# instadeepai/FrameDiPT

Hardware: AMD Instinct MI355X
Metric: residue*diffusion-steps/sec (higher is better)
Workload: dtype fp16

## Files before the change

framedipt_amd/csrc/ipa_proj2.hip:

```cpp
#include <type_traits>

#include "common.hpp"
#include "kernels.hpp"

#define P2_K 256
#define P2_KS (P2_K / 16)
#define P2_WBLK (4 * P2_KS * 1024)
#define P2_XROW (P2_K * 2)
#define P2_LDS (2 * P2_WBLK)

typedef const __attribute__((address_space(3))) float* p2_lds_f32;

#define P2S_HALF 32768
#define P2S_STAGE (2 * P2S_HALF)
#define P2S_BIAS_OFF (2 * P2S_STAGE)
__host__ __device__ __forceinline__ int p2p_src_col(int n) {
  const int c = n >> 7, col = n & 127;
  if (c < 4) {
    if (col < 72) { const int vh = col / 36, r = col % 36; return 192 + (r % 3) * 160 + (2 * c + vh) * 20 + 8 + r / 3; }
    if (col < 120) { const int r = col - 72, kh = r / 24, q = r % 24; return 192 + (q % 3) * 160 + (2 * c + kh) * 20 + q / 3; }
    return -1;
  }
  if (c > 5 || col >= 96) return -1;
  const int hq = col / 24, r = col % 24;
  return (r % 3) * 64 + (4 * (c - 4) + hq) * 8 + r / 3;
}
#define P2P_COLS 768
typedef __attribute__((address_space(3))) f32x4* p2_lds_f32x4w;
typedef __attribute__((address_space(3))) u16x8* p2_lds_u16x8w;
typedef const __attribute__((address_space(3))) unsigned* p2_lds_u32;

__device__ __forceinline__ void p2_kpf_units(const ProjArgs& a, const float (&kv)[24], bool lv, int b, int h, int key, int ntl) {
#pragma unroll
  for (int un = 0; un < 8; ++un) {
    const int f = un >> 1, hf = un & 1;
    unsigned short o[8];
    if (f == 3 && hf == 1) {
      float kn = 0.f;
      if (lv)
#pragma unroll
        for (int c = 0; c < 24; ++c) kn = fmaf(kv[c], kv[c], kn);
      const float m = lv ? a.res_mask[(long)b * a.N + key] : 0.f;
      const float t0 = fmaxf(-0.5f * a.gamma[h] * kn, -65000.f);
      const unsigned short p0 = f2f16(t0);
      const float t1 = t0 - f162f(p0);
      const unsigned short p1 = f2f16(t1);
      const unsigned short p2 = f2f16(t1 - f162f(p1));
      o[0] = f2f16(2.f * m); o[1] = f2f16(m); o[2] = f2f16(lv ? 0.f : -60000.f); o[3] = p0; o[4] = p1; o[5] = p2; o[6] = o[7] = 0;
    } else {
      const int c0 = f < 2 ? 8 * hf : 16;
      const bool lo = f == 1 || (f == 2 && hf == 1);
#pragma unroll
      for (int e = 0; e < 8; ++e) {
        const float x = lv ? kv[c0 + e] : 0.f;
        const unsigned short xh = f2f16(x);
        o[e] = lo ? f2f16(x - f162f(xh)) : xh;
      }
    }
    const u32x4 val = {o[0] | ((unsigned)o[1] << 16), o[2] | ((unsigned)o[3] << 16), o[4] | ((unsigned)o[5] << 16), o[6] | ((unsigned)o[7] << 16)};
    *(u32x4*)(a.kpf + ((((((long)b * a.H + h) * ntl + (key >> 5)) * FD_KPF_FRAGS + f) * 64 + hf * 32 + (key & 31)) << 3)) = val;
  }
}

template <class RQ>
__device__ __forceinline__ void p2_points_walk(const ProjArgs& a, const hx8 (&Af)[P2_KS], const hx8 (&Al)[P2_KS], int n_class, int nq, int walker,
                                               int n_walkers, unsigned lds0, unsigned fr, RQ& request_half) {
  const int tid = threadIdx.x, lane = tid & 63, wave = tid >> 6, li = lane & 31, hi = lane >> 5;
  const int M = a.B * a.N, m0 = blockIdx.x * 256, H = a.H, ntl = a.Np >> 5, ks = a.Np >> 4;
  auto tile_at = [&](int col, int rg) { return lds0 + (unsigned)(col * 1024 + ((rg ^ (col & 63)) << 4)); };
  auto rotate = [&](int row, float px, float py, float pz, float* g3) {
    float R[12];
#pragma unroll
    for (int i = 0; i < 12; ++i) R[i] = *(p2_lds_f32)(unsigned long)(fr + 4 * (i * 256 + row));
    g3[0] = R[0] * px + R[1] * py + R[2] * pz + R[9];
    g3[1] = R[3] * px + R[4] * py + R[5] * pz + R[10];
    g3[2] = R[6] * px + R[7] * py + R[8] * pz + R[11];
  };
  for (int k = walker; k < n_class; k += n_walkers) {
    const int c = nq + k;
    const bool frames = k == walker && tid < 256;
    f32x4 fq = {0.f, 0.f, 0.f, 0.f};
    float ft[3] = {0.f, 0.f, 0.f};
    if (frames) {
      const int gr = m0 + tid < M ? m0 + tid : M - 1;
      fq = *(const f32x4*)(a.quat + (long)gr * 4);
#pragma unroll
      for (int d = 0; d < 3; ++d) ft[d] = a.trans[(long)gr * 3 + d];
    }
    __syncthreads();
    request_half(c, 0, 0);
    request_half(c, 1, 1);
#pragma unroll 1
    for (int half = 0; half < 2; ++half) {
      if (half == 0) __builtin_amdgcn_s_waitcnt(0x0F78);
      else __builtin_amdgcn_s_waitcnt(0x0F70);
      if (half == 0 && frames) {
        const float w = fq[0], x = fq[1], y = fq[2], z = fq[3];
        float R[9];
        R[0] = w * w + x * x - y * y - z * z; R[1] = 2 * x * y - 2 * w * z; R[2] = 2 * x * z + 2 * w * y;
        R[3] = 2 * x * y + 2 * w * z; R[4] = w * w - x * x + y * y - z * z; R[5] = 2 * y * z - 2 * w * x;
        R[6] = 2 * x * z - 2 * w * y; R[7] = 2 * y * z + 2 * w * x; R[8] = w * w - x * x - y * y + z * z;
#pragma unroll
        for (int i = 0; i < 12; ++i) *(__attribute__((address_space(3))) float*)(unsigned long)(fr + 4 * (i * 256 + tid)) = i < 9 ? R[i] : ft[i - 9];
        if (walker == 0 && m0 + tid < M)
#pragma unroll
          for (int i = 0; i < 9; ++i) a.rot[(long)(m0 + tid) * 9 + i] = R[i];
      }
      __syncthreads();
      f32x16 acc[2];
#pragma unroll
      for (int j = 0; j < 2; ++j) {
#pragma unroll
        for (int r = 0; r < 16; ++r) acc[j][r] = 0.f;
        const unsigned wbh = lds0 + half * P2S_STAGE + j * (P2_KS * 1024) + lane * 16, wbl = wbh + P2S_HALF;
        constexpr int DEPTH = 3;
        hx8 wh[DEPTH], wl[DEPTH];
#pragma unroll
        for (int s = 0; s < DEPTH - 1; ++s) { wh[s] = fd_frag(wbh + s * 1024); wl[s] = fd_frag(wbl + s * 1024); }
        __builtin_amdgcn_sched_barrier(0);
#pragma unroll
        for (int s = 0; s < P2_KS; ++s) {
          if (s + DEPTH - 1 < P2_KS) {
            wh[(s + DEPTH - 1) % DEPTH] = fd_frag(wbh + (s + DEPTH - 1) * 1024);
            wl[(s + DEPTH - 1) % DEPTH] = fd_frag(wbl + (s + DEPTH - 1) * 1024);
          }
          const hx8 h = wh[s % DEPTH], l = wl[s % DEPTH];
          acc[j] = fd_mfma32(Af[s], l, acc[j]);
          acc[j] = fd_mfma32(Al[s], h, acc[j]);
          acc[j] = fd_mfma32(Af[s], h, acc[j]);
          __builtin_amdgcn_sched_barrier(0);
        }
      }
      float bv[2];
#pragma unroll
      for (int j = 0; j < 2; ++j) bv[j] = *(p2_lds_f32)(unsigned long)(lds0 + P2S_BIAS_OFF + 4 * (c * 128 + 64 * half + 32 * j + li));
      __syncthreads();
#pragma unroll
      for (int j = 0; j < 2; ++j)
#pragma unroll
        for (int g = 0; g < 4; ++g) {
          const f32x4 v = {acc[j][4 * g] + bv[j], acc[j][4 * g + 1] + bv[j], acc[j][4 * g + 2] + bv[j], acc[j][4 * g + 3] + bv[j]};
          *(p2_lds_f32x4w)(unsigned long)tile_at(64 * half + 32 * j + li, 8 * wave + 2 * g + hi) = v;
        }
    }
    __syncthreads();
    auto tv = [&](int row, int col) { return *(p2_lds_f32)(unsigned long)(tile_at(col, row >> 2) + 4 * (row & 3)); };
    int tid = threadIdx.x;
    asm volatile("" : "+v"(tid));
    if (k < 4) {
      {
        const int row = tid & 255, kh = tid >> 8, m = m0 + row;
        if (m < M) {
          const int b = m / a.N, key = m - b * a.N;
          float kv[24];
#pragma unroll
          for (int e = 0; e < 8; ++e) {
            const int col = 72 + 24 * kh + 3 * e;
            rotate(row, tv(row, col), tv(row, col + 1), tv(row, col + 2), kv + 3 * e);
          }
          p2_kpf_units(a, kv, true, b, 2 * k + kh, key, ntl);
        }
        const int npad = a.Np - a.N;
        if (npad > 0)
          for (int bs = m0 / a.N; bs < a.B && bs * a.N < m0 + 256; ++bs) {
            const int end = bs * a.N + a.N - 1;
            if (end < m0 || end >= m0 + 256) continue;
            float z[24];
#pragma unroll
            for (int q = 0; q < 24; ++q) z[q] = 0.f;
#pragma unroll 1
            for (int u = tid; u < 2 * npad; u += 512) p2_kpf_units(a, z, false, bs, 2 * k + (u & 1), a.N + (u >> 1), ntl);
          }
      }
#pragma unroll 1
      for (int t = tid; t < 64 * 24; t += 512) {
        const int k4 = t & 63, rest = t >> 6, vh = rest / 12, e = rest - 12 * vh, mg = m0 + 4 * k4;
        if (mg >= M) continue;
        const int b = mg / a.N, key = mg - b * a.N, pp = (key & ~15) + fd_perm16(key & 15), h = 2 * k + vh;
        f32x4 pc[3];
#pragma unroll
        for (int d = 0; d < 3; ++d) pc[d] = *(fd_lds_f32x4)(unsigned long)tile_at(36 * vh + 3 * e + d, k4);
        unsigned short vhs[3][4], vls[3][4];
#pragma unroll
        for (int q = 0; q < 4; ++q) {
          float g3[3];
          rotate(4 * k4 + q, pc[0][q], pc[1][q], pc[2][q], g3);
#pragma unroll
          for (int d = 0; d < 3; ++d) {
            const unsigned short vh16 = f2h(g3[d]);
            vhs[d][q] = vh16;
            vls[d][q] = f2h(g3[d] - h2f(vh16));
          }
        }
#pragma unroll
        for (int d = 0; d < 3; ++d) {
          const int rw = 3 * e + d, rl = 36 + rw;
          const long bh3 = ((long)b * H + h) * 3;
          const long oh = ((((bh3 + (rw >> 5)) * ks + (pp >> 4)) * 64 + ((pp >> 3) & 1) * 32 + (rw & 31)) << 3) + (pp & 7);
          const long ol = ((((bh3 + (rl >> 5)) * ks + (pp >> 4)) * 64 + ((pp >> 3) & 1) * 32 + (rl & 31)) << 3) + (pp & 7);
          *(u32x2*)(a.vpt + oh) = u32x2{vhs[d][0] | ((unsigned)vhs[d][1] << 16), vhs[d][2] | ((unsigned)vhs[d][3] << 16)};
          *(u32x2*)(a.vpt + ol) = u32x2{vls[d][0] | ((unsigned)vls[d][1] << 16), vls[d][2] | ((unsigned)vls[d][3] << 16)};
        }
      }
    } else {
#pragma unroll 1
      for (int t = tid; t < 1024; t += 512) {
        const int row = t & 255, hq = t >> 8, m = m0 + row;
        if (m >= M) continue;
        float g[24];
#pragma unroll
        for (int e = 0; e < 8; ++e) {
          const int col = 24 * hq + 3 * e;
          rotate(row, tv(row, col), tv(row, col + 1), tv(row, col + 2), g + 3 * e);
        }
        float* dst = a.qp + ((long)m * H * 8 + (4 * (k - 4) + hq) * 8) * 3;
#pragma unroll
        for (int v = 0; v < 6; ++v) *(f32x4*)(dst + 4 * v) = f32x4{g[4 * v], g[4 * v + 1], g[4 * v + 2], g[4 * v + 3]};
      }
    }
  }
}

__device__ __forceinline__ void p2_node_rows(const ProjArgs& a, const hx8 (&Af)[P2_KS], const hx8 (&Al)[P2_KS], int walker, int n_walkers,
                                             unsigned lds0) {
  const int tid = threadIdx.x, lane = tid & 63, wave = tid >> 6, li = lane & 31, hi = lane >> 5;
  const int M = a.B * a.N, mw = blockIdx.x * 256 + wave * 32, ntl = a.Np >> 5;
  for (int p = walker; p < 3; p += n_walkers) {
    if (p == 0) {
      const int m = mw + li;
      if (m < M) {
        const int b = m / a.N, r = m - b * a.N;
        half_t* dst = a.Kb + ((((long)b * ntl + (r >> 5)) * 16) * 64 + hi * 32 + (r & 31)) * 8;
#pragma unroll
        for (int s = 0; s < P2_KS; ++s) *(hx8*)(dst + s * 64 * 8) = Af[s];
      }
      continue;
    }
    __syncthreads();
    const unsigned xl = lds0 + wave * (32 * P2_XROW);
#pragma unroll
    for (int s = 0; s < P2_KS; ++s)
      *(p2_lds_u16x8w)(unsigned long)(xl + li * P2_XROW + (((2 * s + hi) ^ (li & 15)) << 4)) = __builtin_bit_cast(u16x8, p == 1 ? Af[s] : Al[s]);
    __builtin_amdgcn_s_waitcnt(0xC07F);
    half_t* img = p == 1 ? a.Vt : a.Vt_lo;
#pragma unroll 4
    for (int t = 0; t < 16; ++t) {
      const int task = t * 64 + lane, cc = 2 * (task & 127), k4 = task >> 7, mg = mw + 4 * k4;
      unsigned w[4];
#pragma unroll
      for (int q = 0; q < 4; ++q) {
        const int rr = 4 * k4 + q;
        w[q] = *(p2_lds_u32)(unsigned long)(xl + rr * P2_XROW + (((cc >> 3) ^ (rr & 15)) << 4) + (cc & 7) * 2);
      }
      if (mg >= M) continue;
      const int b = mg / a.N, key = mg - b * a.N, pp = (key & ~15) + fd_perm16(key & 15);
      const long u0 = ((((long)b * 8 + (cc >> 5)) * (2 * ntl) + (pp >> 4)) * 64 + ((pp >> 3) & 1) * 32 + (cc & 31)) * 8 + (pp & 7);
      *(u32x2*)(img + u0) = u32x2{(w[0] & 0xffffu) | (w[1] << 16), (w[2] & 0xffffu) | (w[3] << 16)};
      *(u32x2*)(img + u0 + 8) = u32x2{(w[0] >> 16) | (w[1] & 0xffff0000u), (w[2] >> 16) | (w[3] & 0xffff0000u)};
    }
  }
}

template <bool QK, bool SPLIT>
__device__ __forceinline__ void ipa_proj2_body(const ProjArgs& a, int n_cblk, int walker, int n_walkers, char* smem) {
  const unsigned lds0 = (unsigned)(unsigned long)(__attribute__((address_space(3))) char*)smem;
  const int tid = threadIdx.x, lane = tid & 63, wave = tid >> 6, li = lane & 31, hi = lane >> 5;
  constexpr int RB = SPLIT ? 256 : 128;
  constexpr int TM = SPLIT ? 1 : 2;
  constexpr int NTH = SPLIT ? 512 : FD_THREADS;
  const int wr = SPLIT ? wave : wave >> 1;
  int wc = SPLIT ? 0 : (wave & 1);
  const bool mrg = a.merged != 0;
  const int M = a.B * a.N, HC = a.H * a.C, NOUT = (mrg ? HC : 3 * HC) + a.PT, ntl = a.Np >> 5;
  const int m0 = blockIdx.x * RB;
  const char* wimg = (const char*)a.W_img;
  const char* wimg_lo = (const char*)a.W_img_lo;
  const int nq = HC / 128, per_head = (2 * a.C) / 128, n_class = mrg ? (QK ? nq : n_cblk - nq) : (QK ? 2 * nq : n_cblk - 2 * nq);
  auto cblk_of = [&](int k) {
    if (mrg) return QK ? k : nq + k;
    if (QK) return k < nq ? k : nq + ((k - nq) / (per_head / 2)) * per_head + (k - nq) % (per_head / 2);
    const int nv = nq;
    return k < nv ? nq + (k / (per_head / 2)) * per_head + per_head / 2 + k % (per_head / 2) : 3 * nq + (k - nv);
  };
  int kb = walker;
  auto request = [&](int c, int buf) {
    const char* src = wimg + (size_t)c * P2_WBLK;
#pragma unroll
    for (int u = 0; u < P2_WBLK / (FD_THREADS * 16); ++u)
      fd_dma16(src + (size_t)(u * FD_THREADS + tid) * 16, lds0 + buf * P2_WBLK + (unsigned)(u * FD_THREADS + (tid & ~63)) * 16);
  };
  auto request_half = [&](int c, int half, int buf) {
    const size_t so = (size_t)c * P2_WBLK + (size_t)half * P2S_HALF;
#pragma unroll
    for (int u = 0; u < P2S_HALF / (NTH * 16); ++u) {
      const unsigned d = lds0 + buf * P2S_STAGE + (unsigned)(u * NTH + (tid & ~63)) * 16;
      fd_dma16(wimg + so + (size_t)(u * NTH + tid) * 16, d);
      fd_dma16(wimg_lo + so + (size_t)(u * NTH + tid) * 16, d + P2S_HALF);
    }
  };
  FD_STAMP(0);
  if (!SPLIT && kb < n_class) request(cblk_of(kb), 0);
  hx8 Af[TM][P2_KS];
  hx8 Al[1][SPLIT ? P2_KS : 1];
  if constexpr (SPLIT) {
    f32x4 xv[32];
#pragma unroll
    for (int r = 0; r < 32; ++r) {
      const int gr = m0 + wave * 32 + r < M ? m0 + wave * 32 + r : M - 1;
      xv[r] = *(const f32x4*)(a.A + (long)gr * a.lda + 4 * lane);
    }
    {
      float* bls = (float*)(smem + P2S_BIAS_OFF);
      constexpr int NBV = 16;
      float bv[NBV];
#pragma unroll
      for (int k = 0; k < NBV; ++k) {
        const int v = tid + k * NTH;
        bv[k] = v < NOUT ? a.bias[v] : 0.f;
      }
#pragma unroll
      for (int k = 0; k < NBV; ++k)
        if (tid + k * NTH < n_cblk * 128) bls[tid + k * NTH] = bv[k];
    }
    char* xs = smem + wave * (32 * P2_XROW);
    const unsigned xl = lds0 + wave * (32 * P2_XROW);
#pragma unroll
    for (int pass = 0; pass < 2; ++pass) {
#pragma unroll
      for (int r = 0; r < 32; ++r) {
        f32x4 x = xv[r];
        if (pass) {
#pragma unroll
          for (int q = 0; q < 4; ++q) x[q] -= h2f(f2h(x[q]));
        }
        const u32x2 h = {fd_cvt_pk(x[0], x[1]), fd_cvt_pk(x[2], x[3])};
        *(u32x2*)(xs + r * P2_XROW + (((lane >> 1) ^ (r & 15)) << 4) + 8 * (lane & 1)) = h;
      }
      __builtin_amdgcn_s_waitcnt(0xC07F);
#pragma unroll
      for (int s = 0; s < P2_KS; ++s) {
        const hx8 f = fd_frag(xl + li * P2_XROW + (((2 * s + hi) ^ (li & 15)) << 4));
        if (pass == 0) Af[0][s] = f;
        else Al[0][s] = f;
      }
      __builtin_amdgcn_s_waitcnt(0xC07F);
    }
    __syncthreads();
  } else {
    char* xs = smem + P2_WBLK;
#pragma unroll
    for (int it = 0; it < 32; ++it) {
      const int idx = tid + it * FD_THREADS, r = idx >> 6, c4 = idx & 63;
      const int gr = m0 + r < M ? m0 + r : M - 1;
      const f32x4 x = *(const f32x4*)(a.A + (long)gr * a.lda + 4 * c4);
      const u32x2 h = {fd_cvt_pk(x[0], x[1]), fd_cvt_pk(x[2], x[3])};
      *(u32x2*)(xs + r * P2_XROW + (((c4 >> 1) ^ (r & 15)) << 4) + 8 * (c4 & 1)) = h;
    }
    __syncthreads();
#pragma unroll
    for (int i = 0; i < 2; ++i)
#pragma unroll
      for (int s = 0; s < P2_KS; ++s) {
        const int r = (wr * 2 + i) * 32 + li;
        Af[i][s] = fd_frag(lds0 + P2_WBLK + r * P2_XROW + (((2 * s + hi) ^ (r & 15)) << 4));
      }
    __builtin_amdgcn_s_waitcnt(0xC07F);
  }
  FD_STAMP(1);
  if constexpr (SPLIT && !QK) {
    if (a.pts_img) {
      p2_points_walk(a, Af[0], Al[0], n_class, nq, kb, n_walkers, lds0, lds0 + P2S_BIAS_OFF + n_cblk * 512, request_half);
      return;
    }
  }
  int qk_row[TM];
  int v_row[TM][4];
  int p_row[TM][4];
#pragma unroll
  for (int i = 0; i < TM; ++i) {
    const int m = m0 + (wr * TM + i) * 32 + li;
    const int b = m < M ? m / a.N : 0, r = m - b * a.N;
    qk_row[i] = m < M ? ((b * a.H * ntl + (r >> 5)) * (a.C >> 4) * 64 + (r & 31)) * 8 : -1;
#pragma unroll
    for (int g = 0; g < 4; ++g) {
      const int mg = m0 + (wr * TM + i) * 32 + 8 * g + 4 * hi;
      const int bb = mg < M ? mg / a.N : 0, key = mg - bb * a.N, pp = (key & ~15) + fd_perm16(key & 15);
      v_row[i][g] = mg + 3 < M ? (bb * a.H * (a.C >> 5) * (2 * ntl) + (pp >> 4)) * 512 + ((pp >> 3) & 1) * 256 + (pp & 7) : -1;
      p_row[i][g] = mg + 3 < M ? mg * a.PT : -1;
    }
  }
  auto epi_unit = [&](const f32x16 (&acc)[TM][2], const auto& BQ, const int (&cpart)[2], int kind, int i, int j, int g) {
    if constexpr (QK) {
      if ((g & 1) || qk_row[i] < 0) return;
      const f32x4 b0 = BQ.q(j, g), b1 = BQ.q(j, g + 1);
      const float sc = kind == 0 ? a.qscale : 1.f;
      const u32x4 o = {fd_cvt_pk((acc[i][j][4 * g] + b0[0]) * sc, (acc[i][j][4 * g + 1] + b0[1]) * sc),
                          fd_cvt_pk((acc[i][j][4 * g + 2] + b0[2]) * sc, (acc[i][j][4 * g + 3] + b0[3]) * sc),
                          fd_cvt_pk((acc[i][j][4 * g + 4] + b1[0]) * sc, (acc[i][j][4 * g + 5] + b1[1]) * sc),
                          fd_cvt_pk((acc[i][j][4 * g + 6] + b1[2]) * sc, (acc[i][j][4 * g + 7] + b1[3]) * sc)};
      half_t* dst = (kind == 0 ? a.Qb : a.Kb) + (long)qk_row[i] + cpart[0] + ((2 * j + (g >> 1)) * 64) * 8;
      *(u32x4*)dst = o;
    } else {
      if (cpart[j] < 0) return;
      const float bv = BQ.s(j);
      float v[4];
#pragma unroll
      for (int q = 0; q < 4; ++q) v[q] = acc[i][j][4 * g + q] + bv;
      if (kind == 2) {
        if (v_row[i][g] < 0) return;
        const u32x2 o = {fd_cvt_pk(v[0], v[1]), fd_cvt_pk(v[2], v[3])};
        *(u32x2*)(a.Vt + (long)v_row[i][g] + cpart[j]) = o;
        if (SPLIT && a.Vt_lo) {
          float w[4];
#pragma unroll
          for (int q = 0; q < 4; ++q) w[q] = v[q] - h2f(f2h(v[q]));
          const u32x2 ol = {fd_cvt_pk(w[0], w[1]), fd_cvt_pk(w[2], w[3])};
          *(u32x2*)(a.Vt_lo + (long)v_row[i][g] + cpart[j]) = ol;
        }
      } else {
        if (p_row[i][g] < 0) return;
        float* dst = a.pts + (long)p_row[i][g] + cpart[j];
#pragma unroll
        for (int q = 0; q < 4; ++q) dst[q * a.PT] = v[q];
      }
    }
  };
  auto col_part = [&](int c, int (&cpart)[2]) {
    const int n0 = c * 128;
    if constexpr (QK) {
      const bool isq = n0 < HC;
      const int nn0 = isq ? n0 : n0 - HC, hh = isq ? nn0 / a.C : nn0 / (2 * a.C), cbase = isq ? nn0 % a.C : nn0 % (2 * a.C);
      cpart[0] = (hh * ntl * (a.C >> 4) * 64 + ((cbase >> 4) + 4 * wc) * 64 + hi * 32) * 8;
      cpart[1] = 0;
      return isq ? 0 : 1;
    } else {
      const bool isv = !mrg && n0 < 3 * HC;
#pragma unroll
      for (int j = 0; j < 2; ++j) {
        const int n = n0 + (wc * 2 + j) * 32 + li;
        if (isv) {
          const int nn = n - HC, hh = nn / (2 * a.C), cc = nn % (2 * a.C) - a.C;
          cpart[j] = (hh * (a.C >> 5) + (cc >> 5)) * (2 * ntl) * 512 + (cc & 31) * 8;
        } else cpart[j] = n < NOUT ? n - (mrg ? HC : 3 * HC) : -1;
      }
      return isv ? 2 : 3;
    }
  };
  if constexpr (SPLIT) {
    struct BiasLds {
      unsigned base; int hi, li;
      __device__ __forceinline__ f32x4 q(int j, int g) const { return *(fd_lds_f32x4)(unsigned long)(base + 4 * (j * 32 + 16 * (g >> 1) + 8 * hi + 4 * (g & 1))); }
      __device__ __forceinline__ float s(int j) const { return *(p2_lds_f32)(unsigned long)(base + 4 * (j * 32 + li)); }
    };
    const int n_hs = kb < n_class ? 2 * ((n_class - 1 - kb) / n_walkers + 1) : 0;
    auto cb_of_hs = [&](int hs) { return cblk_of(kb + (hs >> 1) * n_walkers); };
    if (n_hs > 0) request_half(cb_of_hs(0), 0, 0);
    struct HalfBlock { int cp[2]; int kind; unsigned nb; };
    HalfBlock cur = {{0, 0}, 0, 0u}, prev = {{0, 0}, 0, 0u};
    f32x16 acc[1][2];
    auto quarter = [&](int hs, auto J) {
      constexpr int j = decltype(J)::value;
      if (j == 0) {
        __builtin_amdgcn_s_waitcnt(0x0F70);
        __syncthreads();
        if (hs + 1 < n_hs) request_half(cb_of_hs(hs + 1), (hs + 1) & 1, (hs + 1) & 1);
        prev = cur;
        const int c = cb_of_hs(hs);
        wc = hs & 1;
        cur.kind = col_part(c, cur.cp);
        cur.nb = lds0 + P2S_BIAS_OFF + 4u * (unsigned)(c * 128 + 64 * wc);
      }
      const HalfBlock& ep = j == 0 ? prev : cur;
      const bool has_prev = j == 1 || hs > 0;
      const BiasLds bq = {ep.nb, hi, li};
#pragma unroll
      for (int r = 0; r < 16; ++r) acc[0][j][r] = 0.f;
      const unsigned wbh = lds0 + (hs & 1) * P2S_STAGE + j * (P2_KS * 1024) + lane * 16, wbl = wbh + P2S_HALF;
      constexpr int DEPTH = 3;
      hx8 wh[DEPTH], wl[DEPTH];
#pragma unroll
      for (int s = 0; s < DEPTH - 1; ++s) { wh[s] = fd_frag(wbh + s * 1024); wl[s] = fd_frag(wbl + s * 1024); }
      __builtin_amdgcn_sched_barrier(0);
#pragma unroll
      for (int s = 0; s < P2_KS; ++s) {
        if (s + DEPTH - 1 < P2_KS) {
          wh[(s + DEPTH - 1) % DEPTH] = fd_frag(wbh + (s + DEPTH - 1) * 1024);
          wl[(s + DEPTH - 1) % DEPTH] = fd_frag(wbl + (s + DEPTH - 1) * 1024);
        }
        const hx8 h = wh[s % DEPTH], l = wl[s % DEPTH];
        if constexpr (QK) {
          acc[0][j] = fd_mfma32(l, Af[0][s], acc[0][j]);
          acc[0][j] = fd_mfma32(h, Al[0][s], acc[0][j]);
          acc[0][j] = fd_mfma32(h, Af[0][s], acc[0][j]);
        } else {
          acc[0][j] = fd_mfma32(Af[0][s], l, acc[0][j]);
          acc[0][j] = fd_mfma32(Al[0][s], h, acc[0][j]);
          acc[0][j] = fd_mfma32(Af[0][s], h, acc[0][j]);
        }
        if (has_prev && (s & 3) == 1) epi_unit(acc, bq, ep.cp, ep.kind, 0, j ^ 1, s >> 2);
        __builtin_amdgcn_sched_barrier(0);
      }
    };
    for (int hs = 0; hs < n_hs; ++hs) {
      quarter(hs, std::integral_constant<int, 0>{});
      FD_STAMP(2 + 2 * hs);
      quarter(hs, std::integral_constant<int, 1>{});
      FD_STAMP(3 + 2 * hs);
    }
    if (n_hs > 0) {
      const BiasLds bq = {cur.nb, hi, li};
#pragma unroll
      for (int g = 0; g < 4; ++g) epi_unit(acc, bq, cur.cp, cur.kind, 0, 1, g);
    }
    if constexpr (QK)
      if (a.pts_img) p2_node_rows(a, Af[0], Al[0], walker, n_walkers, lds0);
    FD_STAMP(15);
    return;
  }
  if constexpr (!SPLIT) {
  struct BiasReg {
    f32x4 v[2][4];
    __device__ __forceinline__ f32x4 q(int j, int g) const { return v[j][g]; }
    __device__ __forceinline__ float s(int j) const { return v[j][0][0]; }
  };
  auto load_bias = [&](BiasReg& bq, int n0) {
#pragma unroll
    for (int j = 0; j < 2; ++j)
#pragma unroll
      for (int g = 0; g < 4; ++g) {
        if constexpr (QK) bq.v[j][g] = *(const f32x4*)(a.bias + n0 + (wc * 2 + j) * 32 + 16 * (g >> 1) + 8 * hi + 4 * (g & 1));
        else if (g == 0) {
          const int n = n0 + (wc * 2 + j) * 32 + li;
          bq.v[j][0][0] = n < NOUT ? a.bias[n] : 0.f;
        }
      }
  };
  auto step = [&](f32x16 (&accN)[2][2], BiasReg& bqN, int (&cpN)[2], int& kindN, const f32x16 (&accP)[2][2], const BiasReg& bqP,
                  const int (&cpP)[2], int kindP, int k, bool has_prev, int bufc) {
    __builtin_amdgcn_s_waitcnt(0x0F70);
    __syncthreads();
    if (k + n_walkers < n_class) request(cblk_of(k + n_walkers), bufc ^ 1);
    load_bias(bqN, cblk_of(k) * 128);
    kindN = col_part(cblk_of(k), cpN);
#pragma unroll
    for (int i = 0; i < 2; ++i)
#pragma unroll
      for (int j = 0; j < 2; ++j)
#pragma unroll
        for (int r = 0; r < 16; ++r) accN[i][j][r] = 0.f;
    (void)k;
    const unsigned wb = lds0 + bufc * P2_WBLK + (wc * 2) * (P2_KS * 1024) + lane * 16;
    constexpr int DEPTH = 3;
    hx8 w0[DEPTH], w1[DEPTH];
#pragma unroll
    for (int s = 0; s < DEPTH - 1; ++s) {
      w0[s] = fd_frag(wb + s * 1024);
      w1[s] = fd_frag(wb + (P2_KS + s) * 1024);
    }
    __builtin_amdgcn_sched_barrier(0);
#pragma unroll
    for (int s = 0; s < P2_KS; ++s) {
      if (s + DEPTH - 1 < P2_KS) {
        w0[(s + DEPTH - 1) % DEPTH] = fd_frag(wb + (s + DEPTH - 1) * 1024);
        w1[(s + DEPTH - 1) % DEPTH] = fd_frag(wb + (P2_KS + s + DEPTH - 1) * 1024);
      }
      if constexpr (QK) {
#pragma unroll
        for (int i = 0; i < 2; ++i) {
          accN[i][0] = fd_mfma32(w0[s % DEPTH], Af[i][s], accN[i][0]);
          accN[i][1] = fd_mfma32(w1[s % DEPTH], Af[i][s], accN[i][1]);
        }
      } else {
#pragma unroll
        for (int i = 0; i < 2; ++i) {
          accN[i][0] = fd_mfma32(Af[i][s], w0[s % DEPTH], accN[i][0]);
          accN[i][1] = fd_mfma32(Af[i][s], w1[s % DEPTH], accN[i][1]);
        }
      }
      if (has_prev && s < 8) {
        epi_unit(accP, bqP, cpP, kindP, (2 * s) >> 3, ((2 * s) >> 2) & 1, (2 * s) & 3);
        epi_unit(accP, bqP, cpP, kindP, (2 * s + 1) >> 3, ((2 * s + 1) >> 2) & 1, (2 * s + 1) & 3);
      }
      __builtin_amdgcn_sched_barrier(0);
    }
  };
  f32x16 acc0[2][2], acc1[2][2];
  BiasReg bq0, bq1;
  int cp0[2] = {0, 0}, cp1[2] = {0, 0}, kind0 = 0, kind1 = 0;
  bool has_prev = false;
  int n_step = 0;
  (void)n_step;
  for (;;) {
    if (kb >= n_class) break;
    step(acc0, bq0, cp0, kind0, acc1, bq1, cp1, kind1, kb, has_prev, 0);
    FD_STAMP(2 + n_step); ++n_step;
    has_prev = true;
    kb += n_walkers;
    if (kb >= n_class) {
#pragma unroll
      for (int s = 0; s < 16; ++s) epi_unit(acc0, bq0, cp0, kind0, s >> 3, (s >> 2) & 1, s & 3);
      break;
    }
    step(acc1, bq1, cp1, kind1, acc0, bq0, cp0, kind0, kb, true, 1);
    FD_STAMP(2 + n_step); ++n_step;
    kb += n_walkers;
    if (kb >= n_class) {
#pragma unroll
      for (int s = 0; s < 16; ++s) epi_unit(acc1, bq1, cp1, kind1, s >> 3, (s >> 2) & 1, s & 3);
      break;
    }
  }
  }
}
template <bool SPLIT>
__global__ __launch_bounds__(SPLIT ? 512 : FD_THREADS, 1) void ipa_proj2_kernel(ProjArgs a, int n_cblk, int n_walk_qk) {
  extern __shared__ __attribute__((aligned(16))) char smem[];
  if ((int)blockIdx.y < n_walk_qk) ipa_proj2_body<true, SPLIT>(a, n_cblk, blockIdx.y, n_walk_qk, smem);
  else ipa_proj2_body<false, SPLIT>(a, n_cblk, blockIdx.y - n_walk_qk, gridDim.y - n_walk_qk, smem);
}

__global__ void p2_permute_rows_kernel(half_t* img, int ks, int n_q_tiles, int per_head) {
  const int tile = blockIdx.x / ks, s = blockIdx.x % ks;
  const bool qk = tile < n_q_tiles || ((tile - n_q_tiles) % per_head) < per_head / 2;
  if (!qk) return;
  __shared__ u16x8 buf[64];
  u16x8* frag = (u16x8*)img + ((size_t)tile * ks + s) * 64;
  const int lane = threadIdx.x, rho = lane & 31, half = lane >> 5;
  buf[lane] = frag[lane];
  __syncthreads();
  const int hi = (rho >> 2) & 1, r = (rho & 3) + 4 * (rho >> 3), c = 16 * (r >> 3) + 8 * hi + (r & 7);
  frag[lane] = buf[c + 32 * half];
}
int fd_ipa_proj2_permute_image(void* img, int H, int C, int K, hipStream_t st) {
  if ((C & 31) || (K & 15)) return FDIPT_EINVAL;
  const int n_q = H * C / 32, n_kv = 2 * H * C / 32, ks = K / 16;
  hipLaunchKernelGGL(p2_permute_rows_kernel, dim3((n_q + n_kv) * ks), dim3(64), 0, st, (half_t*)img, ks, n_q, 2 * C / 32);
  FD_CHECK_LAUNCH();
  return FDIPT_OK;
}
int fd_ipa_proj2_permute_image_q(void* img, int H, int C, int K, hipStream_t st) {
  if ((C & 31) || (K & 15)) return FDIPT_EINVAL;
  const int n_q = H * C / 32, ks = K / 16;
  hipLaunchKernelGGL(p2_permute_rows_kernel, dim3(n_q * ks), dim3(64), 0, st, (half_t*)img, ks, n_q, 2 * C / 32);
  FD_CHECK_LAUNCH();
  return FDIPT_OK;
}

__global__ void node_images_kernel(int B, int N, int Np, const float* __restrict__ node, int ld, half_t* __restrict__ Kb,
                                   half_t* __restrict__ Vt, half_t* __restrict__ Vt_lo) {
  constexpr int C = 256;
  const int ntl = Np >> 5;
  const long nk = (long)B * Np * (C / 8), nv = (long)B * (C / 32) * (2 * ntl) * 64;
  for (long u = blockIdx.x * (long)blockDim.x + threadIdx.x; u < nk + nv; u += (long)gridDim.x * blockDim.x) {
    if (u < nk) {
      const int cg = (int)(u % (C / 8));
      const long br = u / (C / 8);
      const int r = (int)(br % Np), b = (int)(br / Np);
      u32x4 o = {0u, 0u, 0u, 0u};
      if (r < N) {
        const float* x = node + ((long)b * N + r) * ld + 8 * cg;
        const f32x4 x0 = *(const f32x4*)x, x1 = *(const f32x4*)(x + 4);
        o = u32x4{fd_cvt_pk(x0[0], x0[1]), fd_cvt_pk(x0[2], x0[3]), fd_cvt_pk(x1[0], x1[1]), fd_cvt_pk(x1[2], x1[3])};
      }
      *(u32x4*)(Kb + ((((long)b * ntl + (r >> 5)) * (C >> 4) + (cg >> 1)) * 64 + (cg & 1) * 32 + (r & 31)) * 8) = o;
    } else {
      const long v = u - nk;
      const int lane = (int)(v & 63), half = lane >> 5, c5 = lane & 31;
      const long f = v >> 6;
      const int s16 = (int)(f % (2 * ntl));
      const long bd = f / (2 * ntl);
      const int dt = (int)(bd % (C / 32)), b = (int)(bd / (C / 32));
      const int cc = 32 * dt + c5;
      float xv[8];
#pragma unroll
      for (int e = 0; e < 8; ++e) {
        const int slot = 8 * half + e, pos = 8 * ((slot >> 2) & 1) + 4 * (slot >> 3) + (slot & 3);
        const int key = 16 * s16 + pos;
        xv[e] = key < N ? node[((long)b * N + key) * ld + cc] : 0.f;
      }
      u32x4 oh, ol;
#pragma unroll
      for (int q = 0; q < 4; ++q) {
        oh[q] = fd_cvt_pk(xv[2 * q], xv[2 * q + 1]);
        ol[q] = fd_cvt_pk(xv[2 * q] - h2f(f2h(xv[2 * q])), xv[2 * q + 1] - h2f(f2h(xv[2 * q + 1])));
      }
      *(u32x4*)(Vt + v * 8) = oh;
      if (Vt_lo) *(u32x4*)(Vt_lo + v * 8) = ol;
    }
  }
}
int fd_node_images(int B, int N, int Np, const float* node, int ld, half_t* Kb, half_t* Vt, half_t* Vt_lo, hipStream_t st) {
  if ((Np & 31) || Np < N || (ld & 3) || !Kb || !Vt) return FDIPT_EINVAL;
  const long units = (long)B * Np * 32 + (long)B * 8 * (Np / 16) * 64;
  hipLaunchKernelGGL(node_images_kernel, dim3((unsigned)((units + 255) / 256)), dim3(256), 0, st, B, N, Np, node, ld, Kb, Vt, Vt_lo);
  FD_CHECK_LAUNCH();
  return FDIPT_OK;
}

__global__ void p2_points_image_kernel(const u16x8* __restrict__ src, const float* __restrict__ sbias, u16x8* __restrict__ dst,
                                       float* __restrict__ dbias, int HC, int ks) {
  const long n_units = (long)(HC + P2P_COLS) / 32 * ks * 64;
  for (long u = blockIdx.x * (long)blockDim.x + threadIdx.x; u < n_units; u += (long)gridDim.x * blockDim.x) {
    const int lane = (int)(u & 63), s = (int)((u >> 6) % ks), t = (int)(u / (64L * ks));
    int n = 32 * t + (lane & 31);
    if (n >= HC) {
      const int o = p2p_src_col(n - HC);
      n = o < 0 ? -1 : HC + o;
    }
    dst[u] = n < 0 ? u16x8{0, 0, 0, 0, 0, 0, 0, 0} : src[((long)(n >> 5) * ks + s) * 64 + (n & 31) + 32 * (lane >> 5)];
    if (s == 0 && lane < 32) {
      const int j = 32 * t + lane;
      dbias[j] = n < 0 ? 0.f : sbias[n];
    }
  }
}
int fd_ipa_proj2_points_cols(int H, int C) { return H * C + P2P_COLS; }
int fd_ipa_proj2_points_image(const void* src_img, const float* src_bias, void* img, float* bias, int H, int C, int K, hipStream_t st) {
  if (H != 8 || C != 256 || (K & 15)) return FDIPT_EINVAL;
  const long units = (long)fd_ipa_proj2_points_cols(H, C) / 32 * (K / 16) * 64;
  hipLaunchKernelGGL(p2_points_image_kernel, dim3((unsigned)((units + 255) / 256)), dim3(256), 0, st, (const u16x8*)src_img, src_bias,
                     (u16x8*)img, bias, H * C, K / 16);
  FD_CHECK_LAUNCH();
  return FDIPT_OK;
}
int fd_ipa_proj2_points_supported(const ProjArgs& a, int Pq, int Pv) {
  return a.merged && a.W_img && a.W_img_lo && a.H == 8 && a.C == 256 && a.K == 256 && Pq == 8 && Pv == 12 &&
         a.PT == 3 * a.H * (2 * Pq + Pv) && (a.N & 3) == 0 && (a.Np & 31) == 0 && a.Np >= a.N && (a.lda & 3) == 0;
}
int fd_ipa_proj2_supported(const ProjArgs& a) {
  const int HC = a.H * a.C;
  return a.K == P2_K && a.W_img && (a.N & 3) == 0 && (a.C % 128) == 0 && (HC % 128) == 0 && (a.lda & 3) == 0 && (a.Np & 31) == 0 && (a.PT & 3) == 0;
}
int fd_ipa_proj2(const ProjArgs& a, hipStream_t st) {
  if (!fd_ipa_proj2_supported(a)) return FDIPT_EINVAL;
  const bool split = a.W_img_lo != nullptr;
  const int M = a.B * a.N, NOUT = (a.merged ? 1 : 3) * a.H * a.C + a.PT;
  const int n_cblk = cdiv(NOUT, 128), n_rblk = cdiv(M, split ? 256 : 128);
  if (a.pts_img && (!split || !a.merged || a.PT != P2P_COLS || a.H != 8 || a.C != 256 || !a.quat || !a.trans || !a.rot || !a.qp || !a.kpf ||
                    !a.vpt || !a.gamma || !a.res_mask || !a.Kb || !a.Vt || !a.Vt_lo))
    return FDIPT_EINVAL;
  const int lds = split ? P2S_BIAS_OFF + n_cblk * 128 * 4 + (a.pts_img ? 12 * 256 * 4 : 0) : P2_LDS;
  if (lds > 160 * 1024 || (split && n_cblk * 128 > 8192)) return FDIPT_ESIZE;
  if (hipFuncSetAttribute(split ? (const void*)ipa_proj2_kernel<true> : (const void*)ipa_proj2_kernel<false>,
                          hipFuncAttributeMaxDynamicSharedMemorySize, lds) != hipSuccess)
    return FDIPT_ELAUNCH;
  int ncg = 256 / n_rblk;
  if (ncg < 2) ncg = 2;
  const int n_qk = (a.merged ? 1 : 2) * (a.H * a.C / 128), n_other = n_cblk - n_qk;
  int wq = (ncg * n_qk * 6 + (n_qk * 6 + n_other * 7) / 2) / (n_qk * 6 + n_other * 7);
  if (wq < 1) wq = 1;
  if (wq > ncg - 1) wq = ncg - 1;
  if (wq > n_qk) wq = n_qk;
  int wo = ncg - wq;
  if (wo > n_other) wo = n_other;
  if (split) hipLaunchKernelGGL(ipa_proj2_kernel<true>, dim3(n_rblk, wq + wo), dim3(512), lds, st, a, n_cblk, wq);
  else hipLaunchKernelGGL(ipa_proj2_kernel<false>, dim3(n_rblk, wq + wo), dim3(FD_THREADS), lds, st, a, n_cblk, wq);
  FD_CHECK_LAUNCH();
  return FDIPT_OK;
}
```

Before: 1.203 million.

## Overlap point rotate/store epilogue with second-half MFMA in points walk

```diff
diff --git a/framedipt_amd/csrc/ipa_proj2.hip b/framedipt_amd/csrc/ipa_proj2.hip
--- a/framedipt_amd/csrc/ipa_proj2.hip
+++ b/framedipt_amd/csrc/ipa_proj2.hip
@@ -15,50 +15,60 @@
 #define P2S_STAGE (2 * P2S_HALF)
 #define P2S_BIAS_OFF (2 * P2S_STAGE)
 __host__ __device__ __forceinline__ int p2p_src_col(int n) {
-  const int c = n >> 7, col = n & 127;
+  const int c = n >> 7, hf = (n >> 6) & 1, col = n & 63;
   if (c < 4) {
-    if (col < 72) { const int vh = col / 36, r = col % 36; return 192 + (r % 3) * 160 + (2 * c + vh) * 20 + 8 + r / 3; }
-    if (col < 120) { const int r = col - 72, kh = r / 24, q = r % 24; return 192 + (q % 3) * 160 + (2 * c + kh) * 20 + q / 3; }
+    if (col < 36) return 192 + (col % 3) * 160 + (2 * c + hf) * 20 + 8 + col / 3;
+    if (col < 60) { const int q = col - 36; return 192 + (q % 3) * 160 + (2 * c + hf) * 20 + q / 3; }
     return -1;
   }
-  if (c > 5 || col >= 96) return -1;
-  const int hq = col / 24, r = col % 24;
+  if (c > 5 || col >= 48) return -1;
+  const int hq = 2 * hf + col / 24, r = col % 24;
   return (r % 3) * 64 + (4 * (c - 4) + hq) * 8 + r / 3;
 }
+#ifdef FD_PROF
+#define P2_WSTAMP(k)                                                                                                   \
+  do {                                                                                                                 \
+    if ((threadIdx.x & 255) == 0)                                                                                      \
+      fd_prof[(((blockIdx.x + gridDim.x * blockIdx.y) + (threadIdx.x >> 8) * 4096) & 8191) * 16 + (k)] =               \
+          (k) >= 14 ? __builtin_amdgcn_s_memrealtime() : __builtin_amdgcn_s_memtime();                                 \
+  } while (0)
+#else
+#define P2_WSTAMP(k) \
+  do {               \
+  } while (0)
+#endif
 #define P2P_COLS 768
 typedef __attribute__((address_space(3))) f32x4* p2_lds_f32x4w;
 typedef __attribute__((address_space(3))) u16x8* p2_lds_u16x8w;
 typedef const __attribute__((address_space(3))) unsigned* p2_lds_u32;
 
-__device__ __forceinline__ void p2_kpf_units(const ProjArgs& a, const float (&kv)[24], bool lv, int b, int h, int key, int ntl) {
-#pragma unroll
-  for (int un = 0; un < 8; ++un) {
-    const int f = un >> 1, hf = un & 1;
+__device__ __forceinline__ void p2_kpf_units(const ProjArgs& a, const float (&kv)[24], bool lv, int b, int h, int key, int ntl, int hf) {
+  float kn = 0.f;
+  if (lv)
+#pragma unroll
+    for (int c = 0; c < 24; ++c) kn = fmaf(kv[c], kv[c], kn);
+  const float m = lv ? a.res_mask[(long)b * a.N + key] : 0.f;
+  const float t0 = fmaxf(-0.5f * a.gamma[h] * kn, -65000.f);
+  const unsigned short p0 = f2f16(t0);
+  const float t1 = t0 - f162f(p0);
+  const unsigned short p1 = f2f16(t1);
+  const unsigned short p2 = f2f16(t1 - f162f(p1));
+  const unsigned short nu[8] = {f2f16(2.f * m), f2f16(m), f2f16(lv ? 0.f : -60000.f), p0, p1, p2, 0, 0};
+  unsigned short* dst = a.kpf + ((((((long)b * a.H + h) * ntl + (key >> 5)) * FD_KPF_FRAGS) * 64 + hf * 32 + (key & 31)) << 3);
+#pragma unroll
+  for (int f = 0; f < 4; ++f) {
     unsigned short o[8];
-    if (f == 3 && hf == 1) {
-      float kn = 0.f;
-      if (lv)
-#pragma unroll
-        for (int c = 0; c < 24; ++c) kn = fmaf(kv[c], kv[c], kn);
-      const float m = lv ? a.res_mask[(long)b * a.N + key] : 0.f;
-      const float t0 = fmaxf(-0.5f * a.gamma[h] * kn, -65000.f);
-      const unsigned short p0 = f2f16(t0);
-      const float t1 = t0 - f162f(p0);
-      const unsigned short p1 = f2f16(t1);
-      const unsigned short p2 = f2f16(t1 - f162f(p1));
-      o[0] = f2f16(2.f * m); o[1] = f2f16(m); o[2] = f2f16(lv ? 0.f : -60000.f); o[3] = p0; o[4] = p1; o[5] = p2; o[6] = o[7] = 0;
-    } else {
-      const int c0 = f < 2 ? 8 * hf : 16;
-      const bool lo = f == 1 || (f == 2 && hf == 1);
-#pragma unroll
-      for (int e = 0; e < 8; ++e) {
-        const float x = lv ? kv[c0 + e] : 0.f;
-        const unsigned short xh = f2f16(x);
-        o[e] = lo ? f2f16(x - f162f(xh)) : xh;
-      }
-    }
-    const u32x4 val = {o[0] | ((unsigned)o[1] << 16), o[2] | ((unsigned)o[3] << 16), o[4] | ((unsigned)o[5] << 16), o[6] | ((unsigned)o[7] << 16)};
-    *(u32x4*)(a.kpf + ((((((long)b * a.H + h) * ntl + (key >> 5)) * FD_KPF_FRAGS + f) * 64 + hf * 32 + (key & 31)) << 3)) = val;
+#pragma unroll
+    for (int e = 0; e < 8; ++e) {
+      const float x = !lv ? 0.f : f >= 2 ? kv[16 + e] : hf ? kv[8 + e] : kv[e];
+      const unsigned short xh = f2f16(x);
+      if (f == 0) o[e] = xh;
+      else if (f == 1) o[e] = f2f16(x - f162f(xh));
+      else if (f == 2) o[e] = hf ? f2f16(x - f162f(xh)) : xh;
+      else o[e] = hf ? nu[e] : xh;
+    }
+    *(u32x4*)(dst + f * 512) = u32x4{o[0] | ((unsigned)o[1] << 16), o[2] | ((unsigned)o[3] << 16), o[4] | ((unsigned)o[5] << 16),
+                                     o[6] | ((unsigned)o[7] << 16)};
   }
 }
 
@@ -66,8 +76,10 @@
 __device__ __forceinline__ void p2_points_walk(const ProjArgs& a, const hx8 (&Af)[P2_KS], const hx8 (&Al)[P2_KS], int n_class, int nq, int walker,
                                                int n_walkers, unsigned lds0, unsigned fr, RQ& request_half) {
   const int tid = threadIdx.x, lane = tid & 63, wave = tid >> 6, li = lane & 31, hi = lane >> 5;
+  const int group = __builtin_amdgcn_readfirstlane(wave >> 2);
   const int M = a.B * a.N, m0 = blockIdx.x * 256, H = a.H, ntl = a.Np >> 5, ks = a.Np >> 4;
   auto tile_at = [&](int col, int rg) { return lds0 + (unsigned)(col * 1024 + ((rg ^ (col & 63)) << 4)); };
+  auto tv = [&](int row, int col) { return *(p2_lds_f32)(unsigned long)(tile_at(col, row >> 2) + 4 * (row & 3)); };
   auto rotate = [&](int row, float px, float py, float pz, float* g3) {
     float R[12];
 #pragma unroll
@@ -75,6 +87,81 @@
     g3[0] = R[0] * px + R[1] * py + R[2] * pz + R[9];
     g3[1] = R[3] * px + R[4] * py + R[5] * pz + R[10];
     g3[2] = R[6] * px + R[7] * py + R[8] * pz + R[11];
+  };
+  auto rotate_store = [&](int k, int hf) {
+    int tid = threadIdx.x;
+    asm volatile("" : "+v"(tid));
+    const int lane = tid & 63, li = lane & 31, hi = lane >> 5, row0 = 32 * (tid >> 6), cb = 64 * hf;
+    if (k < 4) {
+      const int h = 2 * k + hf;
+      {
+        const int row = row0 + li, m = m0 + row;
+        if (m < M) {
+          const int b = m / a.N, key = m - b * a.N;
+          float kv[24];
+#pragma unroll
+          for (int e = 0; e < 8; ++e) {
+            const int col = cb + 36 + 3 * e;
+            rotate(row, tv(row, col), tv(row, col + 1), tv(row, col + 2), kv + 3 * e);
+          }
+          p2_kpf_units(a, kv, true, b, h, key, ntl, hi);
+        }
+        const int npad = a.Np - a.N;
+        if (npad > 0)
+          for (int bs = m0 / a.N; bs < a.B && bs * a.N < m0 + 256; ++bs) {
+            const int end = bs * a.N + a.N - 1;
+            if (end < m0 || end >= m0 + 256) continue;
+            float z[24];
+#pragma unroll
+            for (int q = 0; q < 24; ++q) z[q] = 0.f;
+#pragma unroll 1
+            for (int u = tid; u < 2 * npad; u += 512) p2_kpf_units(a, z, false, bs, h, a.N + (u >> 1), ntl, u & 1);
+          }
+      }
+#pragma unroll 1
+      for (int t = lane; t < 8 * 12; t += 64) {
+        const int k4 = (row0 >> 2) + (t & 7), e = t >> 3, mg = m0 + 4 * k4;
+        if (mg >= M) continue;
+        const int b = mg / a.N, key = mg - b * a.N, pp = (key & ~15) + fd_perm16(key & 15);
+        f32x4 pc[3];
+#pragma unroll
+        for (int d = 0; d < 3; ++d) pc[d] = *(fd_lds_f32x4)(unsigned long)tile_at(cb + 3 * e + d, k4);
+        unsigned short vhs[3][4], vls[3][4];
+#pragma unroll
+        for (int q = 0; q < 4; ++q) {
+          float g3[3];
+          rotate(4 * k4 + q, pc[0][q], pc[1][q], pc[2][q], g3);
+#pragma unroll
+          for (int d = 0; d < 3; ++d) {
+            const unsigned short vh16 = f2h(g3[d]);
+            vhs[d][q] = vh16;
+            vls[d][q] = f2h(g3[d] - h2f(vh16));
+          }
+        }
+#pragma unroll
+        for (int d = 0; d < 3; ++d) {
+          const int rw = 3 * e + d, rl = 36 + rw;
+          const long bh3 = ((long)b * H + h) * 3;
+          const long oh = ((((bh3 + (rw >> 5)) * ks + (pp >> 4)) * 64 + ((pp >> 3) & 1) * 32 + (rw & 31)) << 3) + (pp & 7);
+          const long ol = ((((bh3 + (rl >> 5)) * ks + (pp >> 4)) * 64 + ((pp >> 3) & 1) * 32 + (rl & 31)) << 3) + (pp & 7);
+          *(u32x2*)(a.vpt + oh) = u32x2{vhs[d][0] | ((unsigned)vhs[d][1] << 16), vhs[d][2] | ((unsigned)vhs[d][3] << 16)};
+          *(u32x2*)(a.vpt + ol) = u32x2{vls[d][0] | ((unsigned)vls[d][1] << 16), vls[d][2] | ((unsigned)vls[d][3] << 16)};
+        }
+      }
+    } else {
+      const int row = row0 + li, m = m0 + row;
+      if (m < M) {
+        float g[24];
+#pragma unroll
+        for (int e = 0; e < 8; ++e) {
+          const int col = cb + 24 * hi + 3 * e;
+          rotate(row, tv(row, col), tv(row, col + 1), tv(row, col + 2), g + 3 * e);
+        }
+        float* dst = a.qp + ((long)m * H * 8 + (4 * (k - 4) + 2 * hf + hi) * 8) * 3;
+#pragma unroll
+        for (int v = 0; v < 6; ++v) *(f32x4*)(dst + 4 * v) = f32x4{g[4 * v], g[4 * v + 1], g[4 * v + 2], g[4 * v + 3]};
+      }
+    }
   };
   for (int k = walker; k < n_class; k += n_walkers) {
     const int c = nq + k;
@@ -90,134 +177,73 @@
     __syncthreads();
     request_half(c, 0, 0);
     request_half(c, 1, 1);
+    f32x16 acc[2];
 #pragma unroll 1
-    for (int half = 0; half < 2; ++half) {
-      if (half == 0) __builtin_amdgcn_s_waitcnt(0x0F78);
-      else __builtin_amdgcn_s_waitcnt(0x0F70);
-      if (half == 0 && frames) {
-        const float w = fq[0], x = fq[1], y = fq[2], z = fq[3];
-        float R[9];
-        R[0] = w * w + x * x - y * y - z * z; R[1] = 2 * x * y - 2 * w * z; R[2] = 2 * x * z + 2 * w * y;
-        R[3] = 2 * x * y + 2 * w * z; R[4] = w * w - x * x + y * y - z * z; R[5] = 2 * y * z - 2 * w * x;
-        R[6] = 2 * x * z - 2 * w * y; R[7] = 2 * y * z + 2 * w * x; R[8] = w * w - x * x - y * y + z * z;
-#pragma unroll
-        for (int i = 0; i < 12; ++i) *(__attribute__((address_space(3))) float*)(unsigned long)(fr + 4 * (i * 256 + tid)) = i < 9 ? R[i] : ft[i - 9];
-        if (walker == 0 && m0 + tid < M)
-#pragma unroll
-          for (int i = 0; i < 9; ++i) a.rot[(long)(m0 + tid) * 9 + i] = R[i];
-      }
-      __syncthreads();
-      f32x16 acc[2];
-#pragma unroll
-      for (int j = 0; j < 2; ++j) {
-#pragma unroll
-        for (int r = 0; r < 16; ++r) acc[j][r] = 0.f;
-        const unsigned wbh = lds0 + half * P2S_STAGE + j * (P2_KS * 1024) + lane * 16, wbl = wbh + P2S_HALF;
-        constexpr int DEPTH = 3;
-        hx8 wh[DEPTH], wl[DEPTH];
-#pragma unroll
-        for (int s = 0; s < DEPTH - 1; ++s) { wh[s] = fd_frag(wbh + s * 1024); wl[s] = fd_frag(wbl + s * 1024); }
-        __builtin_amdgcn_sched_barrier(0);
-#pragma unroll
-        for (int s = 0; s < P2_KS; ++s) {
-          if (s + DEPTH - 1 < P2_KS) {
-            wh[(s + DEPTH - 1) % DEPTH] = fd_frag(wbh + (s + DEPTH - 1) * 1024);
-            wl[(s + DEPTH - 1) % DEPTH] = fd_frag(wbl + (s + DEPTH - 1) * 1024);
+    for (int st = 0; st < 4; ++st) {
+      const int half = st & 1;
+      if (st == 3 || (st > 0 && group == st - 1)) rotate_store(k, st == 3);
+      int tq = threadIdx.x;
+      asm volatile("" : "+v"(tq));
+      const int lane = tq & 63, wave = tq >> 6, li = lane & 31, hi = lane >> 5;
+      if (st == 0) {
+        __builtin_amdgcn_s_waitcnt(0x0F78);
+        if (frames) {
+          const float w = fq[0], x = fq[1], y = fq[2], z = fq[3];
+          float R[9];
+          R[0] = w * w + x * x - y * y - z * z; R[1] = 2 * x * y - 2 * w * z; R[2] = 2 * x * z + 2 * w * y;
+          R[3] = 2 * x * y + 2 * w * z; R[4] = w * w - x * x + y * y - z * z; R[5] = 2 * y * z - 2 * w * x;
+          R[6] = 2 * x * z - 2 * w * y; R[7] = 2 * y * z + 2 * w * x; R[8] = w * w - x * x - y * y + z * z;
+#pragma unroll
+          for (int i = 0; i < 12; ++i) *(__attribute__((address_space(3))) float*)(unsigned long)(fr + 4 * (i * 256 + tid)) = i < 9 ? R[i] : ft[i - 9];
+          if (walker == 0 && m0 + tid < M)
+#pragma unroll
+            for (int i = 0; i < 9; ++i) a.rot[(long)(m0 + tid) * 9 + i] = R[i];
+        }
+        __syncthreads();
+      }
+      if (st < 2) {
+#pragma unroll
+        for (int j = 0; j < 2; ++j) {
+#pragma unroll
+          for (int r = 0; r < 16; ++r) acc[j][r] = 0.f;
+          const unsigned wbh = lds0 + half * P2S_STAGE + j * (P2_KS * 1024) + lane * 16, wbl = wbh + P2S_HALF;
+          constexpr int DEPTH = 3;
+          hx8 wh[DEPTH], wl[DEPTH];
+#pragma unroll
+          for (int s = 0; s < DEPTH - 1; ++s) { wh[s] = fd_frag(wbh + s * 1024); wl[s] = fd_frag(wbl + s * 1024); }
+          __builtin_amdgcn_sched_barrier(0);
+#pragma unroll
+          for (int s = 0; s < P2_KS; ++s) {
+            if (s + DEPTH - 1 < P2_KS) {
+              wh[(s + DEPTH - 1) % DEPTH] = fd_frag(wbh + (s + DEPTH - 1) * 1024);
+              wl[(s + DEPTH - 1) % DEPTH] = fd_frag(wbl + (s + DEPTH - 1) * 1024);
+            }
+            const hx8 h = wh[s % DEPTH], l = wl[s % DEPTH];
+            acc[j] = fd_mfma32(Af[s], l, acc[j]);
+            acc[j] = fd_mfma32(Al[s], h, acc[j]);
+            acc[j] = fd_mfma32(Af[s], h, acc[j]);
+            __builtin_amdgcn_sched_barrier(0);
           }
-          const hx8 h = wh[s % DEPTH], l = wl[s % DEPTH];
-          acc[j] = fd_mfma32(Af[s], l, acc[j]);
-          acc[j] = fd_mfma32(Al[s], h, acc[j]);
-          acc[j] = fd_mfma32(Af[s], h, acc[j]);
-          __builtin_amdgcn_sched_barrier(0);
-        }
-      }
-      float bv[2];
-#pragma unroll
-      for (int j = 0; j < 2; ++j) bv[j] = *(p2_lds_f32)(unsigned long)(lds0 + P2S_BIAS_OFF + 4 * (c * 128 + 64 * half + 32 * j + li));
-      __syncthreads();
-#pragma unroll
-      for (int j = 0; j < 2; ++j)
-#pragma unroll
-        for (int g = 0; g < 4; ++g) {
-          const f32x4 v = {acc[j][4 * g] + bv[j], acc[j][4 * g + 1] + bv[j], acc[j][4 * g + 2] + bv[j], acc[j][4 * g + 3] + bv[j]};
-          *(p2_lds_f32x4w)(unsigned long)tile_at(64 * half + 32 * j + li, 8 * wave + 2 * g + hi) = v;
-        }
-    }
-    __syncthreads();
-    auto tv = [&](int row, int col) { return *(p2_lds_f32)(unsigned long)(tile_at(col, row >> 2) + 4 * (row & 3)); };
-    int tid = threadIdx.x;
-    asm volatile("" : "+v"(tid));
-    if (k < 4) {
-      {
-        const int row = tid & 255, kh = tid >> 8, m = m0 + row;
-        if (m < M) {
-          const int b = m / a.N, key = m - b * a.N;
-          float kv[24];
-#pragma unroll
-          for (int e = 0; e < 8; ++e) {
-            const int col = 72 + 24 * kh + 3 * e;
-            rotate(row, tv(row, col), tv(row, col + 1), tv(row, col + 2), kv + 3 * e);
+        }
+      }
+      if (st == 0 || st == 2) {
+        const int ph = st >> 1;
+        float bv[2];
+#pragma unroll
+        for (int j = 0; j < 2; ++j) bv[j] = *(p2_lds_f32)(unsigned long)(lds0 + P2S_BIAS_OFF + 4 * (c * 128 + 64 * ph + 32 * j + li));
+        if (st == 0) __builtin_amdgcn_s_waitcnt(0x0F70);
+        __syncthreads();
+#pragma unroll
+        for (int j = 0; j < 2; ++j)
+#pragma unroll
+          for (int g = 0; g < 4; ++g) {
+            const f32x4 v = {acc[j][4 * g] + bv[j], acc[j][4 * g + 1] + bv[j], acc[j][4 * g + 2] + bv[j], acc[j][4 * g + 3] + bv[j]};
+            *(p2_lds_f32x4w)(unsigned long)tile_at(64 * ph + 32 * j + li, 8 * wave + 2 * g + hi) = v;
           }
-          p2_kpf_units(a, kv, true, b, 2 * k + kh, key, ntl);
-        }
-        const int npad = a.Np - a.N;
-        if (npad > 0)
-          for (int bs = m0 / a.N; bs < a.B && bs * a.N < m0 + 256; ++bs) {
-            const int end = bs * a.N + a.N - 1;
-            if (end < m0 || end >= m0 + 256) continue;
-            float z[24];
-#pragma unroll
-            for (int q = 0; q < 24; ++q) z[q] = 0.f;
-#pragma unroll 1
-            for (int u = tid; u < 2 * npad; u += 512) p2_kpf_units(a, z, false, bs, 2 * k + (u & 1), a.N + (u >> 1), ntl);
-          }
-      }
-#pragma unroll 1
-      for (int t = tid; t < 64 * 24; t += 512) {
-        const int k4 = t & 63, rest = t >> 6, vh = rest / 12, e = rest - 12 * vh, mg = m0 + 4 * k4;
-        if (mg >= M) continue;
-        const int b = mg / a.N, key = mg - b * a.N, pp = (key & ~15) + fd_perm16(key & 15), h = 2 * k + vh;
-        f32x4 pc[3];
-#pragma unroll
-        for (int d = 0; d < 3; ++d) pc[d] = *(fd_lds_f32x4)(unsigned long)tile_at(36 * vh + 3 * e + d, k4);
-        unsigned short vhs[3][4], vls[3][4];
-#pragma unroll
-        for (int q = 0; q < 4; ++q) {
-          float g3[3];
-          rotate(4 * k4 + q, pc[0][q], pc[1][q], pc[2][q], g3);
-#pragma unroll
-          for (int d = 0; d < 3; ++d) {
-            const unsigned short vh16 = f2h(g3[d]);
-            vhs[d][q] = vh16;
-            vls[d][q] = f2h(g3[d] - h2f(vh16));
-          }
-        }
-#pragma unroll
-        for (int d = 0; d < 3; ++d) {
-          const int rw = 3 * e + d, rl = 36 + rw;
-          const long bh3 = ((long)b * H + h) * 3;
-          const long oh = ((((bh3 + (rw >> 5)) * ks + (pp >> 4)) * 64 + ((pp >> 3) & 1) * 32 + (rw & 31)) << 3) + (pp & 7);
-          const long ol = ((((bh3 + (rl >> 5)) * ks + (pp >> 4)) * 64 + ((pp >> 3) & 1) * 32 + (rl & 31)) << 3) + (pp & 7);
-          *(u32x2*)(a.vpt + oh) = u32x2{vhs[d][0] | ((unsigned)vhs[d][1] << 16), vhs[d][2] | ((unsigned)vhs[d][3] << 16)};
-          *(u32x2*)(a.vpt + ol) = u32x2{vls[d][0] | ((unsigned)vls[d][1] << 16), vls[d][2] | ((unsigned)vls[d][3] << 16)};
-        }
-      }
-    } else {
-#pragma unroll 1
-      for (int t = tid; t < 1024; t += 512) {
-        const int row = t & 255, hq = t >> 8, m = m0 + row;
-        if (m >= M) continue;
-        float g[24];
-#pragma unroll
-        for (int e = 0; e < 8; ++e) {
-          const int col = 24 * hq + 3 * e;
-          rotate(row, tv(row, col), tv(row, col + 1), tv(row, col + 2), g + 3 * e);
-        }
-        float* dst = a.qp + ((long)m * H * 8 + (4 * (k - 4) + hq) * 8) * 3;
-#pragma unroll
-        for (int v = 0; v < 6; ++v) *(f32x4*)(dst + 4 * v) = f32x4{g[4 * v], g[4 * v + 1], g[4 * v + 2], g[4 * v + 3]};
-      }
-    }
+      }
+      P2_WSTAMP(2 + st);
+    }
+    P2_WSTAMP(14);
   }
 }
 
@@ -512,9 +538,11 @@
 #pragma unroll
       for (int g = 0; g < 4; ++g) epi_unit(acc, bq, cur.cp, cur.kind, 0, 1, g);
     }
+    P2_WSTAMP(6);
     if constexpr (QK)
       if (a.pts_img) p2_node_rows(a, Af[0], Al[0], walker, n_walkers, lds0);
     FD_STAMP(15);
+    P2_WSTAMP(14);
     return;
   }
   if constexpr (!SPLIT) {
```

Result: no change. 1.197 million (-0.6%).
